# databendlabs/databend

Measured on AMD Instinct MI355X. Metric: rows/s TPC-H Q1 hash-agg, higher is better.
Workload: dtype i64/i128 decimal

## Files before the change

### databend_amd/csrc/gbk_merge_lds.h

```cpp

namespace {

int32_t ensure(void** p, size_t* cap, size_t bytes) {
  if (*cap >= bytes) return DBHIP_OK;
  if (*p) {
    int32_t rc = dbhip_free(*p);
    if (rc) return rc;
    *p = nullptr; *cap = 0;
  }
  size_t want = bytes + (bytes >> 3) + 256;
  int32_t rc = dbhip_alloc(want, p);
  if (rc) { *p = nullptr; return rc; }
  *cap = want;
  return DBHIP_OK;
}

int32_t alloc_table(dbhip_groupby* g, int64_t cap, hipStream_t s) {
  uint64_t* nh = nullptr;
  uint64_t* nr = nullptr;
  int32_t rc = dbhip_alloc((size_t)cap * 8, (void**)&nh);
  if (rc == DBHIP_OK) rc = dbhip_alloc((size_t)cap * g->L.W * 8, (void**)&nr);
  hipError_t e = rc == DBHIP_OK ? hipMemsetAsync(nh, 0, (size_t)cap * 8, s) : hipSuccess;
  if (rc != DBHIP_OK || e != hipSuccess) {
    if (nh) (void)dbhip_free(nh);
// ... 79 lines not shown
  const size_t need = (size_t)(used + extra);
  if (need <= g->arena_cap) return DBHIP_OK;
  size_t want = g->arena_cap ? g->arena_cap * 2 : ((size_t)1 << 20);
  while (want < need) want *= 2;
  uint8_t* na = nullptr;
  int32_t rc = dbhip_alloc(want, (void**)&na);
  if (rc) return rc;
  if (used) DBHIP_CHECK(hipMemcpyAsync(na, g->arena, (size_t)used, hipMemcpyDeviceToDevice, s));
  if (g->arena && layout_has_str_minmax(g->L))
    hipLaunchKernelGGL(gb_pin_strings_kernel, dim3(grid_for(g->cap, 256)), dim3(256), 0, s, g->L, g->slot_hash, g->rows, g->cap,
                       (uint64_t)g->arena, (uint64_t)g->arena + g->arena_cap, 2, na, (int64_t)((intptr_t)na - (intptr_t)g->arena), g->ctrl,
                       (unsigned long long*)nullptr);
  DBHIP_CHECK(hipStreamSynchronize(s));
  if (g->arena) (void)dbhip_free(g->arena);
  g->arena = na;
  g->arena_cap = want;
  return DBHIP_OK;
}
int32_t pin_string_states(dbhip_groupby* g, hipStream_t s) {
  if (!layout_has_str_minmax(g->L)) return DBHIP_OK;
  unsigned long long* acc = (unsigned long long*)&g->ctrl[10];
  DBHIP_CHECK(hipMemsetAsync(acc, 0, 8, s));
  const int grid = grid_for(g->cap, 256);
  hipLaunchKernelGGL(gb_pin_strings_kernel, dim3(grid), dim3(256), 0, s, g->L, g->slot_hash, g->rows, g->cap, (uint64_t)g->arena,
                     (uint64_t)g->arena + g->arena_cap, 0, g->arena, (int64_t)0, g->ctrl, acc);
  DBHIP_LAUNCH_CHECK();
  uint64_t bytes = 0;
  DBHIP_CHECK(hipMemcpyAsync(&bytes, acc, 8, hipMemcpyDeviceToHost, s));
  DBHIP_CHECK(hipStreamSynchronize(s));
  if (bytes == 0) return DBHIP_OK;
  int32_t rc = reserve_arena(g, bytes, s);
  if (rc) return rc;
  hipLaunchKernelGGL(gb_pin_strings_kernel, dim3(grid), dim3(256), 0, s, g->L, g->slot_hash, g->rows, g->cap, (uint64_t)g->arena,
                     (uint64_t)g->arena + g->arena_cap, 1, g->arena, (int64_t)0, g->ctrl, acc);
  DBHIP_LAUNCH_CHECK();
  g->arena_pinned += bytes;
  if (g->arena_pinned < (g->arena_live > ((uint64_t)1 << 20) ? g->arena_live : ((uint64_t)1 << 20))) return DBHIP_OK;
  g->arena_pinned = 0;
  DBHIP_CHECK(hipMemsetAsync(acc, 0, 8, s));
  hipLaunchKernelGGL(gb_pin_strings_kernel, dim3(grid), dim3(256), 0, s, g->L, g->slot_hash, g->rows, g->cap, (uint64_t)g->arena,
                     (uint64_t)g->arena + g->arena_cap, 3, g->arena, (int64_t)0, g->ctrl, acc);
  DBHIP_LAUNCH_CHECK();
  uint64_t two[2] = {0, 0};
  DBHIP_CHECK(hipMemcpyAsync(&two[0], acc, 8, hipMemcpyDeviceToHost, s));
  DBHIP_CHECK(hipMemcpyAsync(&two[1], &g->ctrl[8], 8, hipMemcpyDeviceToHost, s));
  DBHIP_CHECK(hipStreamSynchronize(s));
  g->arena_live = two[0];
  if (two[1] <= 2 * two[0] + ((uint64_t)1 << 20)) return DBHIP_OK;
  size_t want = (size_t)1 << 20;
  while (want < 2 * two[0]) want *= 2;
  uint8_t* na = nullptr;
  if ((rc = dbhip_alloc(want, (void**)&na))) return rc;
  DBHIP_CHECK(hipMemsetAsync(&g->ctrl[8], 0, 8, s));
  hipLaunchKernelGGL(gb_pin_strings_kernel, dim3(grid), dim3(256), 0, s, g->L, g->slot_hash, g->rows, g->cap, (uint64_t)g->arena,
                     (uint64_t)g->arena + g->arena_cap, 4, na, (int64_t)0, g->ctrl, acc);
  DBHIP_LAUNCH_CHECK();
  DBHIP_CHECK(hipStreamSynchronize(s));
  trace("groupby: string arena compacted, %llu bytes in use -> %llu live (capacity %zu -> %zu)",
        (unsigned long long)two[1], (unsigned long long)two[0], g->arena_cap, want);
  (void)dbhip_free(g->arena);
  g->arena = na;
  g->arena_cap = want;
  return DBHIP_OK;
}
int32_t reserve_arena_for_chunk(dbhip_groupby* g, hipStream_t s) {
  uint64_t lb = 0;
  DBHIP_CHECK(hipMemcpyAsync(&lb, &g->ctrl[9], 8, hipMemcpyDeviceToHost, s));
  DBHIP_CHECK(hipStreamSynchronize(s));
  if (lb == 0) return DBHIP_OK;
  g->has_long = 1;
  return reserve_arena(g, lb, s);
}
bool layout_has_strings(const GbLayout& L) { return L.str_w1_mask != 0; }
bool layout_has_wide_minmax(const GbLayout& L);

int32_t merge_rows_unpinned(dbhip_groupby* g, const uint64_t* rows_in, int64_t n, hipStream_t s, const uint64_t* n_dev, const uint64_t* abort_dev,
                            int deferred = 0);
int32_t merge_rows(dbhip_groupby* g, const uint64_t* rows_in, int64_t n, hipStream_t s,
                   const uint64_t* n_dev = nullptr, const uint64_t* abort_dev = nullptr) {
  int32_t rc = merge_rows_unpinned(g, rows_in, n, s, n_dev, abort_dev);
  if (rc == DBHIP_OK && n > 0) rc = pin_string_states(g, s);
  return rc;
}
int32_t merge_rows_unpinned(dbhip_groupby* g, const uint64_t* rows_in, int64_t n, hipStream_t s,
                            const uint64_t* n_dev, const uint64_t* abort_dev, int deferred) {
  if (n == 0) return DBHIP_OK;
  if (n > 0xFFFFFFF0LL) {
    set_error("groupby: more than 2^32 rows in one call");
    return DBHIP_ERR_INVALID;
  }
  int32_t rc;
  if ((rc = ensure((void**)&g->gid, &g->gid_cap, (size_t)n * 4))) return rc;
  if ((rc = ensure((void**)&g->retry, &g->retry_cap, (size_t)n * 4))) return rc;
  const int grid = grid_for(n, 256);
  uint64_t* host_ctrl = pinned_words(0);
  if (!host_ctrl) return DBHIP_ERR_HIP;
  const uint64_t* cur_rows = rows_in;
  int64_t cur_n = n;
  const DevCount dc{n_dev, abort_dev};
  if ((deferred || (g->count_host + n) * 135 <= g->cap * 100) && n <= 256) {
    hipLaunchKernelGGL(gb_merge_small_kernel, dim3(1), dim3(256), 0, s, g->L, cur_rows, cur_n, g->slot_hash, g->rows, g->cap, g->hash_mask, g->gid,
                       g->retry, g->ctrl, dc, g->arena);
    DBHIP_LAUNCH_CHECK();
    if (deferred) return DBHIP_OK;
    DBHIP_CHECK(hipMemcpyAsync(host_ctrl, g->ctrl, 5 * sizeof(uint64_t), hipMemcpyDeviceToHost, s));
    DBHIP_CHECK(hipStreamSynchronize(s));
    g->count_host = (int64_t)host_ctrl[0];
    if (host_ctrl[3] & 2) {
      set_error("groupby: a string key longer than 12 bytes was met; keep the CPU operator for this block");
      return DBHIP_ERR_UNSUPPORTED;
    }
    if (host_ctrl[1]) {
      set_error("groupby: collision chain filled the table during retry; create the table with a larger capacity");
      return DBHIP_ERR_CAPACITY;
    }
    return DBHIP_OK;
  }
  if (deferred || (g->count_host + n) * 135 <= g->cap * 100) {
    DBHIP_CHECK(hipMemsetAsync(&g->ctrl[1], 0, 16, s));
    hipLaunchKernelGGL(gb_probe_kernel, dim3(grid), dim3(256), 0, s, g->L, cur_rows, cur_n, g->slot_hash, g->rows, g->cap,
                       g->hash_mask, g->gid, g->ctrl, dc, g->arena);
    if (deferred == 1 || (!deferred && g->count_host > 0 && g->count_host <= 32 && n <= 65536) || n <= 2048 || layout_has_wide_minmax(g->L))
      hipLaunchKernelGGL(gb_accum_lowcard_kernel, dim3(deferred == 1 && grid > 16 ? 16 : grid), dim3(256), 0, s, g->L, cur_rows, cur_n, g->rows, g->gid, g->retry,
                         g->ctrl, dc, g->arena);
    else
      hipLaunchKernelGGL(gb_accum_kernel, dim3(grid), dim3(256), 0, s, g->L, cur_rows, cur_n, g->rows, g->gid, g->retry, g->ctrl, dc, g->arena);
    hipLaunchKernelGGL(gb_retry_kernel, dim3(1), dim3(64), 0, s, g->L, cur_rows, g->slot_hash, g->rows, g->cap, g->hash_mask,
                       g->gid, g->retry, g->ctrl, g->arena);
    DBHIP_LAUNCH_CHECK();
    if (deferred) return DBHIP_OK;
    DBHIP_CHECK(hipMemcpyAsync(host_ctrl, g->ctrl, 5 * sizeof(uint64_t), hipMemcpyDeviceToHost, s));
    DBHIP_CHECK(hipStreamSynchronize(s));
    g->count_host = (int64_t)host_ctrl[0];
    if (host_ctrl[3] & 2) {
      set_error("groupby: a string key longer than 12 bytes was met; keep the CPU operator for this block");
      return DBHIP_ERR_UNSUPPORTED;
    }
    if (host_ctrl[1]) {
      set_error("groupby: collision chain filled the table during retry; create the table with a larger capacity");
      return DBHIP_ERR_CAPACITY;
    }
    return DBHIP_OK;
  }
  if (n_dev || abort_dev) {
    set_error("groupby: device-side row count needs a table that cannot grow during the merge");
    return DBHIP_ERR_INVALID;
  }
  for (int attempt = 0; attempt < 40; ++attempt) {
    DBHIP_CHECK(hipMemsetAsync(&g->ctrl[1], 0, 16, s));
    hipLaunchKernelGGL(gb_probe_kernel, dim3(grid), dim3(256), 0, s, g->L, cur_rows, cur_n, g->slot_hash,
                       g->rows, g->cap, g->hash_mask, g->gid, g->ctrl, dc, g->arena);
    DBHIP_LAUNCH_CHECK();
    DBHIP_CHECK(hipMemcpyAsync(host_ctrl, g->ctrl, 5 * sizeof(uint64_t), hipMemcpyDeviceToHost, s));
    DBHIP_CHECK(hipStreamSynchronize(s));
    bool too_full = host_ctrl[1] != 0 || (int64_t)host_ctrl[0] * 135 > g->cap * 100;
    if (too_full) {
      if ((rc = grow(g, s))) return rc;
      continue;
    }
    g->count_host = (int64_t)host_ctrl[0];
    if (g->count_host <= 32 || layout_has_wide_minmax(g->L)) {
      hipLaunchKernelGGL(gb_accum_lowcard_kernel, dim3(grid), dim3(256), 0, s, g->L, cur_rows, cur_n,
                         g->rows, g->gid, g->retry, g->ctrl, dc, g->arena);
    } else {
      hipLaunchKernelGGL(gb_accum_kernel, dim3(grid), dim3(256), 0, s, g->L, cur_rows, cur_n, g->rows,
                         g->gid, g->retry, g->ctrl, dc, g->arena);
    }
    hipLaunchKernelGGL(gb_retry_kernel, dim3(1), dim3(64), 0, s, g->L, cur_rows, g->slot_hash, g->rows,
                       g->cap, g->hash_mask, g->gid, g->retry, g->ctrl, g->arena);
    DBHIP_LAUNCH_CHECK();
    DBHIP_CHECK(hipMemcpyAsync(host_ctrl, g->ctrl, 5 * sizeof(uint64_t), hipMemcpyDeviceToHost, s));
    DBHIP_CHECK(hipStreamSynchronize(s));
    g->count_host = (int64_t)host_ctrl[0];
    if (host_ctrl[3] & 2) {
      set_error("groupby: a string key longer than 12 bytes was met; keep the CPU operator for this block");
      return DBHIP_ERR_UNSUPPORTED;
    }
    if (host_ctrl[1] & 2) {
      set_error("groupby: collision chain filled the table during retry; create the table with a larger capacity");
      return DBHIP_ERR_CAPACITY;
    }
    return DBHIP_OK;
// ... 264 lines not shown
```

### databend_amd/csrc/gbk_rows.h

```cpp

namespace {

struct HashCols {
  GbCol c[GB_MAX_KEYS];
  int n;
};

__global__ __launch_bounds__(256) void group_hash_kernel(HashCols hc, int64_t n, uint64_t* out,
                                                         unsigned long long* bad) {
  constexpr int U = 4;
  const int64_t T = (int64_t)gridDim.x * blockDim.x;
  const int64_t t = (int64_t)blockIdx.x * blockDim.x + threadIdx.x;
  for (int64_t base = 0; base < n; base += U * T) {
    int64_t row[U];
    bool in[U];
    uint64_t h[U];
#pragma unroll
    for (int u = 0; u < U; ++u) {
      row[u] = base + u * T + t;
      in[u] = row[u] < n;
      if (!in[u]) row[u] = n - 1;
      h[u] = 0;
    }
    for (int k = 0; k < hc.n; ++k) {
// ... 163 lines not shown
      if (C.arg[a].data != nullptr && C.arg[a].type == DBHIP_T_STRING) {
        const GbCol& ac = C.arg[a];
#pragma unroll
        for (int u = 0; u < U; ++u) {
          const int64_t j = ac.is_scalar ? 0 : row[u];
          valid[u] = !ac.validity || bit_get(ac.validity, ac.voff + j);
          const uint32_t* v = (const uint32_t*)ac.data + 4 * j;
          const uint32_t len = v[0];
          uint64_t ww[2] = {0, 0};
          if (sv_is_inline(len) || !valid[u]) {
            bool vv;
            gb_load_words(ac, row[u], ww, &vv);
          } else if (ac.buffers) {
            ww[0] = ((uint64_t)v[1] << 32) | len;
            ww[1] = (uint64_t)sv_bytes(v, ac.buffers);
          } else {
            atomicOr((unsigned long long*)&ctrl[3], 2ULL);
          }
          w0[u] = ww[0]; w1[u] = ww[1];
        }
      } else if (C.arg[a].data != nullptr) gb_load_words_n<U>(C.arg[a], row, w0, w1, valid);
#pragma unroll
      for (int u = 0; u < U; ++u) {
        if (!in[u]) continue;
        uint64_t* s = rows_in + li[u] * L.W + L.agg_off[a];
        uint64_t v[GB_MAX_STATE_WORDS];
        gb_row_contrib(L, a, w0[u], w1[u], valid[u], v);
        for (int k = 0; k < L.agg_words[a]; ++k) s[k] = v[k];
      }
    }
  }
}

__device__ __forceinline__ uint64_t probe_word(uint64_t h, uint64_t mask) {
  uint64_t hw = h & mask;
  return hw == 0 ? 1 : hw;
}
__device__ __forceinline__ uint64_t home_slot(uint64_t hw, int64_t cap) {
  return hw >> (__builtin_clzll((unsigned long long)cap) + 1);
}

struct DevCount {
  const uint64_t* n_dev;
  const uint64_t* abort_dev;
};
__device__ __forceinline__ int64_t dev_rows(const DevCount& dc, int64_t n) {
  if (dc.abort_dev && (*dc.abort_dev & 7)) return 0;
  if (dc.n_dev) { const int64_t m = (int64_t)*dc.n_dev; return m < n ? m : n; }
  return n;
}

__device__ __forceinline__ bool bytes_equal(const uint8_t* x, const uint8_t* y, uint32_t len) {
  for (uint32_t i = 0; i < len; ++i)
    if (x[i] != y[i]) return false;
  return true;
}
__device__ __forceinline__ bool keys_equal(const GbLayout& L, const uint64_t* a, const uint64_t* b, const uint8_t* arena) {
  bool eq = true;
  for (int k = 0; k < L.nkey_words; ++k) {
    if (((L.str_w1_mask >> k) & 1) && (uint32_t)a[k - 1] > SV_INLINE_MAX) {
      eq = eq && a[k - 1] == b[k - 1] && bytes_equal((const uint8_t*)a[k], arena + b[k], (uint32_t)a[k - 1]);
      continue;
    }
    eq &= (a[k] == b[k]);
  }
  return eq;
}
__device__ __forceinline__ void write_group_keys(const GbLayout& L, const uint64_t* r, uint64_t* d, uint8_t* arena, uint64_t* ctrl) {
  for (int k = 0; k < L.nkey_words; ++k) {
    if (((L.str_w1_mask >> k) & 1) && (uint32_t)r[k - 1] > SV_INLINE_MAX) {
      const uint32_t len = (uint32_t)r[k - 1];
      const unsigned long long off = atomicAdd((unsigned long long*)&ctrl[8], (unsigned long long)((len + 7) & ~7u));
      const uint8_t* src = (const uint8_t*)r[k];
      for (uint32_t i = 0; i < len; ++i) arena[off + i] = src[i];
      d[k] = off;
      continue;
    }
    d[k] = r[k];
  }
}

__device__ __forceinline__ void gb_probe_body(const GbLayout& L, const uint64_t* rows_in, int64_t n,
                                              uint64_t* slot_hash, uint64_t* rows, int64_t cap,
                                              uint64_t hash_mask, uint32_t* gid, uint64_t* ctrl, uint8_t* arena) {
  const uint64_t cmask = (uint64_t)cap - 1;
  __shared__ uint32_t wg_new;
  if (threadIdx.x == 0) wg_new = 0;
  __syncthreads();
  uint32_t my_new = 0;
  for (int64_t i = (int64_t)blockIdx.x * blockDim.x + threadIdx.x; i < n;
       i += (int64_t)gridDim.x * blockDim.x) {
    bool claimed = false;
    {
      const uint64_t* r = rows_in + i * L.W;
      const uint64_t hw = probe_word(r[L.hash_word], hash_mask);
      uint64_t pos = home_slot(hw, cap);
      uint32_t found = GB_INVALID_SLOT;
      for (int64_t step = 0; step < cap; ++step) {
        unsigned long long cur = __hip_atomic_load((unsigned long long*)&slot_hash[pos], __ATOMIC_RELAXED,
                                                   __HIP_MEMORY_SCOPE_AGENT);
        if (cur == 0) {
          unsigned long long old = atomicCAS((unsigned long long*)&slot_hash[pos], 0ULL, (unsigned long long)hw);
          if (old == 0) {
            uint64_t* d = rows + pos * L.W;
            write_group_keys(L, r, d, arena, ctrl);
            d[L.hash_word] = r[L.hash_word];
            for (int a = 0; a < L.naggs; ++a) gb_state_identity(L, a, d + L.agg_off[a]);
            claimed = true;
            found = (uint32_t)pos;
            break;
          }
          cur = old;
        }
        if (cur == hw) {
          found = (uint32_t)pos;
          break;
        }
        pos = (pos + 1) & cmask;
      }
      if (found == GB_INVALID_SLOT) atomicOr((unsigned long long*)&ctrl[1], 1ULL);
      gid[i] = found;
    }
    my_new += claimed;
  }
  my_new = (uint32_t)wave_sum_u64(my_new);
  if (lane_id() == 0 && my_new) atomicAdd(&wg_new, my_new);
  __syncthreads();
  if (threadIdx.x == 0 && wg_new) atomicAdd((unsigned long long*)&ctrl[0], (unsigned long long)wg_new);
}
__global__ __launch_bounds__(256) void gb_probe_kernel(GbLayout L, const uint64_t* rows_in, int64_t n,
                                                       uint64_t* slot_hash, uint64_t* rows, int64_t cap,
                                                       uint64_t hash_mask, uint32_t* gid, uint64_t* ctrl, DevCount dc, uint8_t* arena) {
  gb_probe_body(L, rows_in, dev_rows(dc, n), slot_hash, rows, cap, hash_mask, gid, ctrl, arena);
}

__global__ __launch_bounds__(256) void gb_accum_kernel(GbLayout L, const uint64_t* rows_in, int64_t n,
                                                       uint64_t* rows, const uint32_t* gid,
                                                       uint32_t* retry, uint64_t* ctrl, DevCount dc, const uint8_t* arena) {
  n = dev_rows(dc, n);
  for (int64_t i = (int64_t)blockIdx.x * blockDim.x + threadIdx.x; i < n;
       i += (int64_t)gridDim.x * blockDim.x) {
    const uint64_t* r = rows_in + i * L.W;
    uint32_t pos = gid[i];
    uint64_t* d = rows + (uint64_t)pos * L.W;
    if (!keys_equal(L, r, d, arena)) {
      unsigned long long k = atomicAdd((unsigned long long*)&ctrl[2], 1ULL);
      retry[k] = (uint32_t)i;
      continue;
    }
    for (int a = 0; a < L.naggs; ++a) gb_atomic_merge(L, a, d + L.agg_off[a], r + L.agg_off[a]);
  }
}

__device__ __forceinline__ uint64_t wave_min_u64(uint64_t v) {
#pragma unroll
  for (int off = 32; off >= 1; off >>= 1) {
    uint64_t o = __shfl_xor(v, off, 64);
    v = o < v ? o : v;
  }
  return v;
}
__device__ __forceinline__ uint64_t wave_max_u64(uint64_t v) {
#pragma unroll
  for (int off = 32; off >= 1; off >>= 1) {
    uint64_t o = __shfl_xor(v, off, 64);
    v = o > v ? o : v;
  }
  return v;
}
__device__ __forceinline__ double wave_sum_f64(double v) {
#pragma unroll
  for (int off = 32; off >= 1; off >>= 1) v += __shfl_xor(v, off, 64);
  return v;
}

__device__ __forceinline__ void gb_accum_lowcard_body(const GbLayout& L, const uint64_t* rows_in,
                                                      int64_t n, uint64_t* rows,
                                                      const uint32_t* gid, uint32_t* retry,
                                                      uint64_t* ctrl, const uint8_t* arena) {
  const int64_t n_pad = (n + 63) & ~63LL;
  for (int64_t i = (int64_t)blockIdx.x * blockDim.x + threadIdx.x; i < n_pad;
       i += (int64_t)gridDim.x * blockDim.x) {
    bool active = i < n;
    const uint64_t* r = rows_in + (active ? i : 0) * L.W;
    uint32_t pos = active ? gid[i] : GB_INVALID_SLOT;
    if (active) {
      const uint64_t* d = rows + (uint64_t)pos * L.W;
      if (!keys_equal(L, r, d, arena)) {
        unsigned long long k = atomicAdd((unsigned long long*)&ctrl[2], 1ULL);
        retry[k] = (uint32_t)i;
        active = false;
      }
    }
    uint64_t todo = __ballot(active);
    while (todo) {
      int leader = __ffsll((long long)todo) - 1;
      uint32_t lpos = __shfl(pos, leader, 64);
      bool mine = active && pos == lpos;
      uint64_t m = __ballot(mine);
      uint64_t* d = rows + (uint64_t)lpos * L.W;
      for (int a = 0; a < L.naggs; ++a) {
        const uint64_t* v = r + L.agg_off[a];
        uint64_t out[GB_MAX_STATE_WORDS] = {0, 0, 0, 0};
        if (gb_minmax_str(L, a)) {
          if (mine) gb_minmax_str_locked(L.agg_kind[a] == DBHIP_AGG_MIN, d + L.agg_off[a], v);
          continue;
        }
        if (gb_sum256(L, a) || gb_minmax256(L, a)) {
          if (mine) gb_atomic_merge(L, a, d + L.agg_off[a], v);
          continue;
        }
        switch (L.agg_kind[a]) {
          case DBHIP_AGG_COUNT:
            out[0] = wave_sum_u64(mine ? v[0] : 0);
            break;
          case DBHIP_AGG_SUM:
            if (L.agg_flag[a]) out[L.agg_flag[a]] = wave_max_u64(mine ? v[L.agg_flag[a]] : 0);
            if (L.agg_words[a] - (L.agg_flag[a] ? 1 : 0) == 3) {
              u128 t = mine ? (((u128)v[1] << 64) | v[0]) : (u128)0;
              uint64_t e = mine ? v[2] : 0;
#pragma unroll
              for (int off = 32; off >= 1; off >>= 1) {
                uint64_t olo = __shfl_xor((uint64_t)t, off, 64), ohi = __shfl_xor((uint64_t)(t >> 64), off, 64);
                uint64_t oe = __shfl_xor(e, off, 64);
                u128 o = ((u128)ohi << 64) | olo;
                u128 r = t + o;
                e += oe + (r < t ? 1 : 0);
                t = r;
              }
              out[0] = (uint64_t)t;
              out[1] = (uint64_t)(t >> 64);
              out[2] = e;
            } else if (L.agg_type[a] == DBHIP_T_F32 || L.agg_type[a] == DBHIP_T_F64) {
              out[0] = (uint64_t)__double_as_longlong(
                  wave_sum_f64(mine ? __longlong_as_double((long long)v[0]) : 0.0));
            } else {
              out[0] = wave_sum_u64(mine ? v[0] : 0);
            }
            break;
          case DBHIP_AGG_MIN:
            out[0] = wave_min_u64((mine && v[1]) ? v[0] : ~0ULL);
            out[1] = wave_max_u64(mine ? v[1] : 0);
            if (L.agg_words[a] == 3) out[2] = wave_min_u64((mine && v[1] && v[0] == out[0]) ? v[2] : ~0ULL);
            break;
          default:
            out[0] = wave_max_u64((mine && v[1]) ? v[0] : 0ULL);
            out[1] = wave_max_u64(mine ? v[1] : 0);
            if (L.agg_words[a] == 3) out[2] = wave_max_u64((mine && v[1] && v[0] == out[0]) ? v[2] : 0ULL);
            break;
        }
        if (lane_id() == leader) gb_atomic_merge(L, a, d + L.agg_off[a], out);
      }
      todo &= ~m;
    }
  }
}
__global__ __launch_bounds__(256) void gb_accum_lowcard_kernel(GbLayout L, const uint64_t* rows_in,
                                                               int64_t n, uint64_t* rows,
                                                               const uint32_t* gid, uint32_t* retry,
                                                               uint64_t* ctrl, DevCount dc, const uint8_t* arena) {
  gb_accum_lowcard_body(L, rows_in, dev_rows(dc, n), rows, gid, retry, ctrl, arena);
}

__device__ __forceinline__ void gb_retry_body(const GbLayout& L, const uint64_t* rows_in, uint64_t* slot_hash, uint64_t* rows,
                                              int64_t cap, uint64_t hash_mask, const uint32_t* gid,
                                              const uint32_t* retry, uint64_t* ctrl, uint8_t* arena) {
  const uint64_t cmask = (uint64_t)cap - 1;
  const uint64_t nretry = ctrl[2];
  for (uint64_t t = 0; t < nretry; ++t) {
    const uint32_t i = retry[t];
    const uint64_t* r = rows_in + (uint64_t)i * L.W;
    const uint64_t hw = probe_word(r[L.hash_word], hash_mask);
    uint64_t pos = ((uint64_t)gid[i] + 1) & cmask;
    bool done = false;
    for (int64_t step = 0; step < cap && !done; ++step) {
      uint64_t cur = slot_hash[pos];
      uint64_t* d = rows + pos * L.W;
      if (cur == 0) {
        if ((int64_t)(ctrl[0] + 1) * 135 > cap * 100) break;
        slot_hash[pos] = hw;
        write_group_keys(L, r, d, arena, ctrl);
        d[L.hash_word] = r[L.hash_word];
        for (int a = 0; a < L.naggs; ++a) gb_state_identity(L, a, d + L.agg_off[a]);
        ctrl[0] += 1;
        cur = hw;
      }
      if (cur == hw && keys_equal(L, r, d, arena)) {
        for (int a = 0; a < L.naggs; ++a) gb_atomic_merge(L, a, d + L.agg_off[a], r + L.agg_off[a]);
        done = true;
      }
      pos = (pos + 1) & cmask;
    }
    if (!done) ctrl[1] |= 2;
  }
}
__global__ void gb_retry_kernel(GbLayout L, const uint64_t* rows_in, uint64_t* slot_hash, uint64_t* rows,
                                int64_t cap, uint64_t hash_mask, const uint32_t* gid,
                                const uint32_t* retry, uint64_t* ctrl, uint8_t* arena) {
  if (threadIdx.x != 0 || blockIdx.x != 0) return;
  gb_retry_body(L, rows_in, slot_hash, rows, cap, hash_mask, gid, retry, ctrl, arena);
}

__global__ __launch_bounds__(256) void gb_merge_small_kernel(GbLayout L, const uint64_t* rows_in, int64_t n, uint64_t* slot_hash, uint64_t* rows,
                                                             int64_t cap, uint64_t hash_mask, uint32_t* gid, uint32_t* retry, uint64_t* ctrl,
                                                             DevCount dc, uint8_t* arena) {
  n = dev_rows(dc, n);
  if (threadIdx.x < 2) ctrl[1 + threadIdx.x] = 0;
  __threadfence();
  __syncthreads();
  gb_probe_body(L, rows_in, n, slot_hash, rows, cap, hash_mask, gid, ctrl, arena);
  __threadfence();
  __syncthreads();
  gb_accum_lowcard_body(L, rows_in, n, rows, gid, retry, ctrl, arena);
  __threadfence();
  __syncthreads();
  if (threadIdx.x == 0) gb_retry_body(L, rows_in, slot_hash, rows, cap, hash_mask, gid, retry, ctrl, arena);
}

__global__ __launch_bounds__(256) void gb_rehash_kernel(GbLayout L, const uint64_t* old_hash,
                                                        const uint64_t* old_rows, int64_t old_cap,
                                                        uint64_t* new_hash, uint64_t* new_rows,
                                                        int64_t new_cap, uint64_t hash_mask) {
  const uint64_t cmask = (uint64_t)new_cap - 1;
  for (int64_t s = (int64_t)blockIdx.x * blockDim.x + threadIdx.x; s < old_cap;
       s += (int64_t)gridDim.x * blockDim.x) {
    uint64_t hw = old_hash[s];
    if (hw == 0) continue;
    const uint64_t* r = old_rows + s * L.W;
    uint64_t pos = home_slot(probe_word(r[L.hash_word], hash_mask), new_cap);
    while (true) {
      unsigned long long old = atomicCAS((unsigned long long*)&new_hash[pos], 0ULL, (unsigned long long)hw);
      if (old == 0) break;
      pos = (pos + 1) & cmask;
    }
    uint64_t* d = new_rows + pos * L.W;
    for (int k = 0; k < L.W; ++k) d[k] = r[k];
  }
}

__global__ __launch_bounds__(256) void gb_flush_kernel(GbLayout L, const uint64_t* slot_hash,
                                                       const uint64_t* rows, int64_t cap,
                                                       uint64_t* out_rows, int64_t max_rows, uint64_t* ctrl) {
  __shared__ uint32_t wtot[4];
  __shared__ unsigned long long base_s;
  const int tid = threadIdx.x, lane = tid & 63, wave = tid >> 6;
  const int64_t nchunks = (cap + 2047) / 2048;
  for (int64_t c = blockIdx.x; c < nchunks; c += gridDim.x) {
    const int64_t s0 = c * 2048 + (int64_t)tid * 8;
    uint32_t occ = 0;
#pragma unroll
    for (int k = 0; k < 8; ++k)
      if (s0 + k < cap && slot_hash[s0 + k] != 0) occ |= 1u << k;
    const uint32_t mine = (uint32_t)__popc(occ);
    uint32_t incl = mine;
#pragma unroll
    for (int d = 1; d < 64; d <<= 1) { const uint32_t o = __shfl_up(incl, d, 64); if (lane >= d) incl += o; }
    if (lane == 63) wtot[wave] = incl;
    __syncthreads();
    uint32_t wbase = 0, all = 0;
#pragma unroll
    for (int w = 0; w < 4; ++w) { if (w < wave) wbase += wtot[w]; all += wtot[w]; }
    if (tid == 0 && all) base_s = atomicAdd((unsigned long long*)&ctrl[4], (unsigned long long)all);
    __syncthreads();
    if (all) {
      uint64_t idx = base_s + wbase + incl - mine;
#pragma unroll
      for (int k = 0; k < 8; ++k) {
        if (!((occ >> k) & 1)) continue;
        if ((int64_t)idx < max_rows) {
          const uint64_t* r = rows + (s0 + k) * L.W;
          uint64_t* d = out_rows + idx * L.W;
          for (int q = 0; q < L.W; ++q) d[q] = r[q];
        }
        ++idx;
      }
    }
    __syncthreads();
  }
}

__global__ __launch_bounds__(64) void gb_block_header_kernel(uint64_t* block, int W, int64_t max_rows, const uint64_t* ctrl) {
  const int t = threadIdx.x;
  if (t < W) block[t] = t == 0 ? ((int64_t)ctrl[4] > max_rows ? ~0ULL : ctrl[4]) : 0;
}

__global__ __launch_bounds__(256) void gb_compact_blocks_kernel(const uint64_t* __restrict__ blocks, int64_t stride_words, int W,
                                                                int skip, uint64_t* __restrict__ out, uint64_t* __restrict__ xst = nullptr,
                                                                int n_blocks = 0, int64_t max_rows = 0, int check_w1 = 0) {
  const int b = blockIdx.x;
  if (xst) {
    uint64_t total = 0;
    int bad = 0;
    for (int p = 0; p < n_blocks; ++p) {
      const uint64_t c = blocks[(int64_t)p * stride_words];
      if (c == ~0ULL || (int64_t)c > max_rows || (check_w1 && blocks[(int64_t)p * stride_words + 1] != 0)) { if (!bad) bad = p + 1; }
      else if (p != skip) total += c;
    }
    if (b == 0 && threadIdx.x == 0) { xst[0] = bad ? 0 : total; xst[1] = bad ? 1 : 0; xst[2] = (uint64_t)bad; }
    if (bad) return;
// ... 433 lines not shown
```

### databend_amd/csrc/k_fagg.hip

```cpp
#include "fagg_device.h"
#include "runtime.h"

#include <dirent.h>
#include <dlfcn.h>
#include <errno.h>
#include <sys/stat.h>
#include <fcntl.h>
#include <signal.h>
#include <spawn.h>
#include <sys/wait.h>
#include <unistd.h>

#include <atomic>
#include <chrono>
#include <deque>
#include <map>
#include <mutex>
#include <string>

#include <stdlib.h>
#include <string.h>
#include <time.h>

using namespace dbhip;
// ... 875 lines not shown
    }
    put(prog->arg_regs, (size_t)L.naggs * 4);
    const char hf = filter_bitmap != nullptr;
    put(&hf, 1);
    int sh = -1;
    for (int i = (int)pp->shapes.size() - 1; i >= 0 && sh < 0; --i)
      if (pp->shapes[(size_t)i].sig == sig) sh = i;
    if (sh < 0) {
      FaShape S;
      FaArgs A;
      memset(&A, 0, sizeof(A));
      bool may_raise = false;
      const int32_t rc = fa_build_args(L, keys, prog, A, &S.general, &S.nwords, &may_raise);
      if (rc) return rc;
      A.has_filter = filter_bitmap != nullptr;
      S.lds = (size_t)(A.P.n_slots > 6 ? A.P.n_slots : 6) * FA_ROWS * 256 * 8;
      if (S.lds > 60 * 1024) {
        set_error("dbhip_groupby_add_block_program: %d live LDS slots exceed the register file; split the expression", A.P.n_slots);
        return DBHIP_ERR_UNSUPPORTED;
      }
      fa_shape(A, S.A);
      S.sig = sig;
      pp->shapes.push_back(std::move(S));
      sh = (int)pp->shapes.size() - 1;
    }
    FaPending P;
    memset(&P.b, 0, sizeof(P.b));
    P.shape = sh;
    for (int c = 0; c < prog->n_inputs; ++c) {
      P.b.in_data[c] = prog->inputs[c].data; P.b.in_valid[c] = prog->inputs[c].validity; P.b.in_voff[c] = prog->inputs[c].validity_offset;
    }
    for (int k = 0; k < L.nkeys; ++k) { P.b.key_data[k] = keys[k].data; P.b.key_valid[k] = keys[k].validity; P.b.key_voff[k] = keys[k].validity_offset; }
    P.b.filter_bits = filter_bitmap; P.b.filter_off = filter_bit_offset; P.b.n = n;
    pp->bound = true; pp->stream = s;
    return fa_pipe_enqueue(g, pp, P, s);
  }
  FaArgs A;
  memset(&A, 0, sizeof(A));
  bool general = false, may_raise = false;
  int nwords = 0;
  int32_t rc = fa_build_args(L, keys, prog, A, &general, &nwords, &may_raise);
  if (rc) return rc;
  A.filter_bits = filter_bitmap; A.filter_off = filter_bit_offset; A.n = n;
  A.has_filter = filter_bitmap != nullptr;
  const size_t lds = (size_t)(A.P.n_slots > 6 ? A.P.n_slots : 6) * FA_ROWS * 256 * 8;
  if (lds > 60 * 1024) {
    set_error("dbhip_groupby_add_block_program: %d live LDS slots exceed the register file; split the expression", A.P.n_slots);
    return DBHIP_ERR_UNSUPPORTED;
  }
  const int64_t nchunks = ceil_div(n, 64 * FA_ROWS);
  const int grid = (int)(ceil_div(nchunks, 4) < 512 ? ceil_div(nchunks, 4) : 512);
  if (FaPipe* pp = (FaPipe*)*dbhip_groupby_pipe_slot_internal(g); pp && !t_prepare_only) {
    int64_t committed = 0;
    if ((rc = fa_pipe_checkpoint(g, pp, &committed, true))) return rc;
  }
  const size_t rows_bytes = (size_t)grid * FA_MAX_SLOTS * L.W * 8;
  uint8_t* ws = (uint8_t*)scratch(rows_bytes + 64, 6, s);
  if (!ws) return DBHIP_ERR_HIP;
  uint64_t* ctrl = (uint64_t*)ws;
  A.ctrl = ctrl;
  A.partial_rows = (uint64_t*)(ws + 64);
  A.P.err_words = nullptr;
  A.P.err_count = (unsigned long long*)&ctrl[2];
  uint64_t* host_ctrl = pinned_words(1);
  if (!host_ctrl) return DBHIP_ERR_HIP;
  host_ctrl[0] = host_ctrl[1] = host_ctrl[2] = 0;
  const int64_t n_max = (int64_t)grid * FA_MAX_SLOTS;
  const bool chained = (dbhip_groupby_count_internal(g) + n_max) * 135 <= dbhip_groupby_capacity_internal(g) * 100;
  if ((rc = dbhip_groupby_reserve_merge_internal(g, n_max))) return rc;
  if (t_prepare_only) {
    (void)jit_kernel(A, dbhip_groupby_count_internal(g) > 4 ? 8 : 4, general, nwords, JIT_COMPILE);
    if (FaPipe* pq = (FaPipe*)*dbhip_groupby_pipe_slot_internal(g); pq && pq->on)
      (void)jit_kernel(A, dbhip_groupby_count_internal(g) > 4 ? 8 : 4, general, nwords, JIT_COMPILE, nullptr, true);
    return DBHIP_OK;
  }
  for (int variant = dbhip_groupby_count_internal(g) > 4 ? 1 : 0; variant < 2; ++variant) {
    DBHIP_CHECK(hipMemsetAsync(ctrl, 0, 64, s));
    kernel_timer_start(s);
    if ((rc = fa_launch(A, variant == 0 ? 4 : 8, general, nwords, grid, lds, s))) return rc;
    kernel_timer_stop(s);
    DBHIP_LAUNCH_CHECK();
    DBHIP_CHECK(hipMemcpyAsync(host_ctrl, ctrl, 24, hipMemcpyDeviceToHost, s));
    if (chained && !may_raise) {
      rc = dbhip_groupby_merge_rows_dev_internal(g, A.partial_rows, n_max, &ctrl[0], &ctrl[1], s);
      if (rc) return rc;
      if (!(host_ctrl[1] & 3)) return DBHIP_OK;
    } else {
      DBHIP_CHECK(hipStreamSynchronize(s));
    }
    if (!(host_ctrl[1] & 1)) break;
  }
  if (host_ctrl[1] & 2) {
    set_error("dbhip_groupby_add_block_program: a group key string is longer than 12 bytes");
    return DBHIP_ERR_UNSUPPORTED;
  }
  if (host_ctrl[1] & 1) {
    set_error("dbhip_groupby_add_block_program: more than %d distinct groups inside one workgroup; use the operator-at-a-time path", FA_MAX_SLOTS);
    return DBHIP_ERR_CAPACITY;
  }
  if (host_ctrl[2]) {
    set_error("dbhip_groupby_add_block_program: %llu row error(s) in the fused maps (Decimal overflow / divided by zero); "
              "evaluate the maps with dbhip_expr_eval to get the rows", (unsigned long long)host_ctrl[2]);
    return DBHIP_ERR_ROW_ERRORS;
  }
  return dbhip_groupby_merge_rows_internal(g, A.partial_rows, (int64_t)host_ctrl[0], s);
}

int32_t dbhip_groupby_set_pipelined(dbhip_groupby* g, int32_t on, void* stream) {
  DBHIP_REQUIRE(g, "dbhip_groupby_set_pipelined: NULL argument");
  void** slot = dbhip_groupby_pipe_slot_internal(g);
  FaPipe* pp = (FaPipe*)*slot;
  if (!on) {
    if (!pp) return DBHIP_OK;
    int64_t committed = 0;
    const int32_t rc = fa_pipe_checkpoint(g, pp, &committed, true);
    pp->on = false; pp->bound = false;
    return rc;
  }
  const GbLayout& L = *dbhip_groupby_layout_internal(g);
  if (!dbhip_fagg_layout_ok_internal(L)) {
    set_error("dbhip_groupby_set_pipelined: layout outside the fused kernel (<= %d key words, <= %d aggregates, <= %d state words)", FA_KW, FA_MAXA, FA_MAXW);
    return DBHIP_ERR_UNSUPPORTED;
  }
  if (pp) { pp->on = true; return DBHIP_OK; }
  pp = new (std::nothrow) FaPipe();
  DBHIP_REQUIRE(pp, "dbhip_groupby_set_pipelined: out of host memory");
  hipStream_t s = resolve_stream(stream);
  pp->cap_rows = 65536;
  int32_t rc = dbhip_alloc((size_t)pp->cap_rows * L.W * 8, (void**)&pp->rows);
  hipError_t e = rc == DBHIP_OK ? hipMalloc((void**)&pp->ctrl, 64) : hipSuccess;
  if (rc == DBHIP_OK && e == hipSuccess) e = hipHostMalloc((void**)&pp->status_host, 64, hipHostMallocMapped);
  if (rc == DBHIP_OK && e == hipSuccess) e = hipHostGetDevicePointer((void**)&pp->status_dev, pp->status_host, 0);
  if (rc == DBHIP_OK && e == hipSuccess) { memset(pp->status_host, 0, 64); e = hipMemsetAsync(pp->ctrl, 0, 64, s); }
  if (rc == DBHIP_OK && e == hipSuccess) e = hipStreamSynchronize(s);
  for (int i = 0; i < FA_PIPE_RING && rc == DBHIP_OK && e == hipSuccess; ++i) {
    e = hipHostMalloc((void**)&pp->tab_host[i], FA_PIPE_TABLE_BYTES, hipHostMallocDefault);
    if (e == hipSuccess) e = hipMalloc((void**)&pp->tab_dev[i], FA_PIPE_TABLE_BYTES);
    if (e == hipSuccess) e = hipEventCreateWithFlags(&pp->tab_ev[i], hipEventDisableTiming);
  }
  if (rc == DBHIP_OK && e == hipSuccess) rc = dbhip_groupby_reserve_merge_internal(g, pp->cap_rows);
  if (rc != DBHIP_OK || e != hipSuccess) {
    dbhip_fagg_pipe_destroy_internal(pp);
    return rc != DBHIP_OK ? rc : hip_fail(e, "dbhip_groupby_set_pipelined");
  }
  pp->count_seen = dbhip_groupby_count_internal(g);
  pp->on = true;
  *slot = pp;
  return DBHIP_OK;
}

int32_t dbhip_groupby_checkpoint(dbhip_groupby* g, int64_t* out_blocks_committed_host, void* stream) {
  DBHIP_REQUIRE(g, "dbhip_groupby_checkpoint: NULL argument");
  if (out_blocks_committed_host) *out_blocks_committed_host = 0;
  FaPipe* pp = (FaPipe*)*dbhip_groupby_pipe_slot_internal(g);
  if (!pp) return DBHIP_OK;
  if (pp->bound && stream && pp->stream != resolve_stream(stream)) {
    set_error("dbhip_groupby_checkpoint: the table's blocks were queued on another stream");
    return DBHIP_ERR_INVALID;
  }
  const int32_t rc = fa_pipe_checkpoint(g, pp, out_blocks_committed_host, true);
  pp->bound = false;
  return rc;
}

int32_t dbhip_groupby_prepare_program(dbhip_groupby* g, const dbhip_col* keys, const dbhip_agg_program* prog) {
  t_prepare_only = true;
  const int32_t rc = dbhip_groupby_add_block_program(g, keys, prog, 1, nullptr, 0, nullptr);
// ... 146 lines not shown
```

Measured before the change: 89.07 billion.

## Add LDS fold-merge kernel that pre-aggregates partial rows before global hash merge

Adds a single-workgroup merge kernel with 1024 threads. It first folds the incoming partial rows into a small LDS hash table, word by word with LDS atomics, then probes and accumulates only the distinct folded groups (plus any unfolded overflow rows) into the global hash table. This is meant to replace many global atomic merges on few groups with cheap LDS atomics, and it prefetches input words into registers. The chained fused-agg path also passes a tighter row bound for the 4-slot variant. The cost is more kernel complexity, a large LDS footprint, and carry-propagation logic for multiword sums.

New measurement: 89.31 billion (median of 6 runs). No clear change (+0.3%).

```diff
diff --git a/databend_amd/csrc/gbk_merge_lds.h b/databend_amd/csrc/gbk_merge_lds.h
--- a/databend_amd/csrc/gbk_merge_lds.h
+++ b/databend_amd/csrc/gbk_merge_lds.h
@@ -185,6 +185,31 @@
   if (rc == DBHIP_OK && n > 0) rc = pin_string_states(g, s);
   return rc;
 }
+struct FmShape { int lcap, n_cap; size_t lds; };
+bool fold_merge_shape(const GbLayout& L, int64_t n, FmShape* out) {
+  if (n > FM_MAX_ROWS || layout_has_wide_minmax(L)) return false;
+  int lcap = 256;
+  while (lcap >= 8 && (size_t)lcap * L.W * 8 > 40 * 1024) lcap >>= 1;
+  if (lcap < 8) return false;
+  out->lcap = lcap;
+  out->n_cap = (int)n;
+  out->lds = 8 * ((size_t)lcap * L.W + 2 * (size_t)lcap) + 4 * ((size_t)((L.W + 1) & ~1) + (size_t)lcap) + 2 * (2 * (size_t)lcap + 2 * (size_t)((n + 3) & ~3LL));
+  return out->lds <= 60 * 1024;
+}
+int32_t merge_read_back(dbhip_groupby* g, uint64_t* host_ctrl, hipStream_t s) {
+  DBHIP_CHECK(hipMemcpyAsync(host_ctrl, g->ctrl, 5 * sizeof(uint64_t), hipMemcpyDeviceToHost, s));
+  DBHIP_CHECK(hipStreamSynchronize(s));
+  g->count_host = (int64_t)host_ctrl[0];
+  if (host_ctrl[3] & 2) {
+    set_error("groupby: a string key longer than 12 bytes was met; keep the CPU operator for this block");
+    return DBHIP_ERR_UNSUPPORTED;
+  }
+  if (host_ctrl[1]) {
+    set_error("groupby: collision chain filled the table during retry; create the table with a larger capacity");
+    return DBHIP_ERR_CAPACITY;
+  }
+  return DBHIP_OK;
+}
 int32_t merge_rows_unpinned(dbhip_groupby* g, const uint64_t* rows_in, int64_t n, hipStream_t s,
                             const uint64_t* n_dev, const uint64_t* abort_dev, int deferred) {
   if (n == 0) return DBHIP_OK;
@@ -201,6 +226,14 @@
   const uint64_t* cur_rows = rows_in;
   int64_t cur_n = n;
   const DevCount dc{n_dev, abort_dev};
+  FmShape fm;
+  if ((deferred || (g->count_host + n) * 135 <= g->cap * 100) && fold_merge_shape(g->L, n, &fm)) {
+    hipLaunchKernelGGL(gb_fold_merge_kernel, dim3(1), dim3(FM_THREADS), fm.lds, s, g->L, cur_rows, cur_n, g->slot_hash, g->rows, g->cap, g->hash_mask,
+                       g->gid, g->retry, g->ctrl, dc, g->arena, fm.lcap, fm.n_cap);
+    DBHIP_LAUNCH_CHECK();
+    if (deferred) return DBHIP_OK;
+    return merge_read_back(g, host_ctrl, s);
+  }
   if ((deferred || (g->count_host + n) * 135 <= g->cap * 100) && n <= 256) {
     hipLaunchKernelGGL(gb_merge_small_kernel, dim3(1), dim3(256), 0, s, g->L, cur_rows, cur_n, g->slot_hash, g->rows, g->cap, g->hash_mask, g->gid,
                        g->retry, g->ctrl, dc, g->arena);
diff --git a/databend_amd/csrc/gbk_rows.h b/databend_amd/csrc/gbk_rows.h
--- a/databend_amd/csrc/gbk_rows.h
+++ b/databend_amd/csrc/gbk_rows.h
@@ -269,7 +269,8 @@
 
 __device__ __forceinline__ void gb_probe_body(const GbLayout& L, const uint64_t* rows_in, int64_t n,
                                               uint64_t* slot_hash, uint64_t* rows, int64_t cap,
-                                              uint64_t hash_mask, uint32_t* gid, uint64_t* ctrl, uint8_t* arena) {
+                                              uint64_t hash_mask, uint32_t* gid, uint64_t* ctrl, uint8_t* arena,
+                                              const uint16_t* idx = nullptr) {
   const uint64_t cmask = (uint64_t)cap - 1;
   __shared__ uint32_t wg_new;
   if (threadIdx.x == 0) wg_new = 0;
@@ -279,7 +280,7 @@
        i += (int64_t)gridDim.x * blockDim.x) {
     bool claimed = false;
     {
-      const uint64_t* r = rows_in + i * L.W;
+      const uint64_t* r = rows_in + (idx ? (int64_t)idx[i] : i) * L.W;
       const uint64_t hw = probe_word(r[L.hash_word], hash_mask);
       uint64_t pos = home_slot(hw, cap);
       uint32_t found = GB_INVALID_SLOT;
@@ -321,13 +322,11 @@
   gb_probe_body(L, rows_in, dev_rows(dc, n), slot_hash, rows, cap, hash_mask, gid, ctrl, arena);
 }
 
-__global__ __launch_bounds__(256) void gb_accum_kernel(GbLayout L, const uint64_t* rows_in, int64_t n,
-                                                       uint64_t* rows, const uint32_t* gid,
-                                                       uint32_t* retry, uint64_t* ctrl, DevCount dc, const uint8_t* arena) {
-  n = dev_rows(dc, n);
+__device__ __forceinline__ void gb_accum_body(const GbLayout& L, const uint64_t* rows_in, int64_t n, uint64_t* rows, const uint32_t* gid,
+                                              uint32_t* retry, uint64_t* ctrl, const uint8_t* arena, const uint16_t* idx = nullptr) {
   for (int64_t i = (int64_t)blockIdx.x * blockDim.x + threadIdx.x; i < n;
        i += (int64_t)gridDim.x * blockDim.x) {
-    const uint64_t* r = rows_in + i * L.W;
+    const uint64_t* r = rows_in + (idx ? (int64_t)idx[i] : i) * L.W;
     uint32_t pos = gid[i];
     uint64_t* d = rows + (uint64_t)pos * L.W;
     if (!keys_equal(L, r, d, arena)) {
@@ -337,6 +336,11 @@
     }
     for (int a = 0; a < L.naggs; ++a) gb_atomic_merge(L, a, d + L.agg_off[a], r + L.agg_off[a]);
   }
+}
+__global__ __launch_bounds__(256) void gb_accum_kernel(GbLayout L, const uint64_t* rows_in, int64_t n,
+                                                       uint64_t* rows, const uint32_t* gid,
+                                                       uint32_t* retry, uint64_t* ctrl, DevCount dc, const uint8_t* arena) {
+  gb_accum_body(L, rows_in, dev_rows(dc, n), rows, gid, retry, ctrl, arena);
 }
 
 __device__ __forceinline__ uint64_t wave_min_u64(uint64_t v) {
@@ -451,12 +455,12 @@
 
 __device__ __forceinline__ void gb_retry_body(const GbLayout& L, const uint64_t* rows_in, uint64_t* slot_hash, uint64_t* rows,
                                               int64_t cap, uint64_t hash_mask, const uint32_t* gid,
-                                              const uint32_t* retry, uint64_t* ctrl, uint8_t* arena) {
+                                              const uint32_t* retry, uint64_t* ctrl, uint8_t* arena, const uint16_t* idx = nullptr) {
   const uint64_t cmask = (uint64_t)cap - 1;
   const uint64_t nretry = ctrl[2];
   for (uint64_t t = 0; t < nretry; ++t) {
     const uint32_t i = retry[t];
-    const uint64_t* r = rows_in + (uint64_t)i * L.W;
+    const uint64_t* r = rows_in + (uint64_t)(idx ? (uint32_t)idx[i] : i) * L.W;
     const uint64_t hw = probe_word(r[L.hash_word], hash_mask);
     uint64_t pos = ((uint64_t)gid[i] + 1) & cmask;
     bool done = false;
@@ -502,6 +506,190 @@
   __threadfence();
   __syncthreads();
   if (threadIdx.x == 0) gb_retry_body(L, rows_in, slot_hash, rows, cap, hash_mask, gid, retry, ctrl, arena);
+}
+
+enum { FM_SKIP = 0, FM_ADD, FM_ADDC, FM_FADD, FM_MIN, FM_MAX, FM_OR };
+constexpr uint32_t FM_NONE = 0xFFFFu;
+constexpr int FM_THREADS = 1024;
+constexpr int64_t FM_MAX_ROWS = 4096;
+
+__device__ __forceinline__ void gb_accum_spread_body(const GbLayout& L, const uint64_t* rows_in, int64_t n, uint64_t* rows, const uint32_t* gid,
+                                                     uint32_t* retry, uint64_t* ctrl, const uint8_t* arena, const uint16_t* idx,
+                                                     uint32_t* any_retry) {
+  const int na = L.naggs > 0 ? L.naggs : 1;
+  const int64_t total = n * na;
+  for (int64_t x = threadIdx.x; x < total; x += blockDim.x) {
+    const int64_t i = x / na;
+    const int a = (int)(x - i * na);
+    const uint64_t* r = rows_in + (idx ? (int64_t)idx[i] : i) * L.W;
+    uint64_t* d = rows + (uint64_t)gid[i] * L.W;
+    if (!keys_equal(L, r, d, arena)) {
+      if (a == 0) {
+        unsigned long long k = atomicAdd((unsigned long long*)&ctrl[2], 1ULL);
+        retry[k] = (uint32_t)i;
+        *any_retry = 1;
+      }
+      continue;
+    }
+    if (a < L.naggs) gb_atomic_merge(L, a, d + L.agg_off[a], r + L.agg_off[a]);
+  }
+}
+
+__device__ __forceinline__ void gb_fold_merge_step(const GbLayout& L, const uint64_t* rows_in, int64_t n, const uint16_t* idx, uint64_t* slot_hash,
+                                                   uint64_t* rows, int64_t cap, uint64_t hash_mask, uint32_t* gid, uint32_t* retry,
+                                                   uint64_t* ctrl, uint8_t* arena, uint32_t* any_retry) {
+  gb_probe_body(L, rows_in, n, slot_hash, rows, cap, hash_mask, gid, ctrl, arena, idx);
+  __syncthreads();
+  gb_accum_spread_body(L, rows_in, n, rows, gid, retry, ctrl, arena, idx, any_retry);
+  __syncthreads();
+  if (threadIdx.x == 0 && *any_retry) {
+    __threadfence();
+    gb_retry_body(L, rows_in, slot_hash, rows, cap, hash_mask, gid, retry, ctrl, arena, idx);
+    ctrl[2] = 0;
+    *any_retry = 0;
+    __threadfence();
+  }
+  __syncthreads();
+}
+
+__device__ __forceinline__ uint64_t gb_fold_word(uint32_t op, uint64_t v, uint64_t* d, const uint64_t* seen) {
+  switch (op) {
+    case FM_ADD:
+      if (v) atomicAdd((unsigned long long*)d, (unsigned long long)v);
+      break;
+    case FM_ADDC:
+      if (v) return atomicAdd((unsigned long long*)d, (unsigned long long)v);
+      break;
+    case FM_FADD:
+      atomicAdd((double*)d, __longlong_as_double((long long)v));
+      break;
+    case FM_MIN:
+      if (*seen) atomicMin((unsigned long long*)d, (unsigned long long)v);
+      break;
+    case FM_MAX:
+      if (*seen) atomicMax((unsigned long long*)d, (unsigned long long)v);
+      break;
+    default:
+      if (v) atomicOr((unsigned long long*)d, 1ULL);
+      break;
+  }
+  return 0;
+}
+__device__ __forceinline__ void gb_fold_carry(uint64_t* d, const uint32_t* lop_w) {
+  for (;;) {
+    ++d; ++lop_w;
+    const uint64_t old = atomicAdd((unsigned long long*)d, 1ULL);
+    if (*lop_w != FM_ADDC || old != ~0ULL) break;
+  }
+}
+
+__global__ __launch_bounds__(FM_THREADS) void gb_fold_merge_kernel(GbLayout L, const uint64_t* __restrict__ rows_in, int64_t n_bound,
+                                                                   uint64_t* slot_hash, uint64_t* rows, int64_t cap, uint64_t hash_mask,
+                                                                   uint32_t* gid, uint32_t* retry, uint64_t* ctrl, DevCount dc, uint8_t* arena,
+                                                                   int lcap, int n_cap) {
+  extern __shared__ uint64_t fm_lds[];
+  __shared__ uint32_t lcount, lnpass, lretry;
+  constexpr int T = FM_THREADS;
+  const int W = L.W, tid = threadIdx.x;
+  uint64_t* lrows = fm_lds;
+  uint64_t* lhash = lrows + (size_t)lcap * W;
+  uint32_t* lop = (uint32_t*)(lhash + 2 * lcap);
+  uint32_t* lgid = lop + ((W + 1) & ~1);
+  uint16_t* lidx = (uint16_t*)(lgid + lcap);
+  uint16_t* eid = lidx + 2 * lcap;
+  uint16_t* pass = eid + n_cap;
+  const uint32_t hmask = 2u * (uint32_t)lcap - 1;
+  const uint32_t cap_words = (uint32_t)n_cap * (uint32_t)W;
+  uint64_t q0 = rows_in[(uint32_t)tid < cap_words ? tid : 0], q1 = rows_in[(uint32_t)(tid + T) < cap_words ? tid + T : 0];
+  uint64_t q2 = rows_in[(uint32_t)(tid + 2 * T) < cap_words ? tid + 2 * T : 0], q3 = rows_in[(uint32_t)(tid + 3 * T) < cap_words ? tid + 3 * T : 0];
+  int64_t n64 = dev_rows(dc, n_bound);
+  const int n = (int)(n64 < (int64_t)n_cap ? n64 : (int64_t)n_cap);
+  if (tid < 2) ctrl[1 + tid] = 0;
+  if (tid == 0) { lcount = 0; lnpass = 0; lretry = 0; }
+  for (int s = tid; s <= (int)hmask; s += T) lhash[s] = 0;
+  for (int w = tid; w < W; w += T) lop[w] = FM_SKIP;
+  __syncthreads();
+  for (int a = tid; a < L.naggs; a += T) {
+    const int off = L.agg_off[a], fw = L.agg_flag[a];
+    switch (L.agg_kind[a]) {
+      case DBHIP_AGG_COUNT:
+        lop[off] = FM_ADD;
+        break;
+      case DBHIP_AGG_SUM: {
+        const int ns = L.agg_words[a] - (fw ? 1 : 0);
+        if (L.agg_type[a] == DBHIP_T_F32 || L.agg_type[a] == DBHIP_T_F64) lop[off] = FM_FADD;
+        else for (int k = 0; k < ns; ++k) lop[off + k] = k + 1 < ns ? FM_ADDC : FM_ADD;
+        if (fw) lop[off + fw] = FM_OR;
+      } break;
+      case DBHIP_AGG_MIN:
+        lop[off] = FM_MIN; lop[off + 1] = FM_OR;
+        break;
+      default:
+        lop[off] = FM_MAX; lop[off + 1] = FM_OR;
+        break;
+    }
+  }
+  __syncthreads();
+
+#pragma nounroll
+  for (int base = 0; base < n; base += T) {
+    const int i = base + tid;
+    const uint64_t* r = rows_in + (size_t)(i < n ? i : 0) * W;
+    uint32_t slot = FM_NONE;
+    if (i < n) {
+      const uint64_t hw = probe_word(r[L.hash_word], hash_mask);
+      uint32_t pos = (uint32_t)(hw ^ (hw >> 29)) & hmask;
+      for (uint32_t step = 0; step <= hmask; ++step) {
+        uint64_t cur = ((volatile uint64_t*)lhash)[pos];
+        if (cur == 0) {
+          const unsigned long long old = atomicCAS((unsigned long long*)&lhash[pos], 0ULL, (unsigned long long)hw);
+          if (old == 0) {
+            const uint32_t e = atomicAdd(&lcount, 1u);
+            if (e < (uint32_t)lcap) {
+              uint64_t* d = lrows + (size_t)e * W;
+              for (int k = 0; k < L.nkey_words; ++k) d[k] = r[k];
+              d[L.hash_word] = r[L.hash_word];
+              for (int a = 0; a < L.naggs; ++a) gb_state_identity(L, a, d + L.agg_off[a]);
+            }
+            lidx[pos] = (uint16_t)(e < (uint32_t)lcap ? e : FM_NONE);
+            slot = pos;
+            break;
+          }
+          cur = old;
+        }
+        if (cur == hw) { slot = pos; break; }
+        pos = (pos + 1) & hmask;
+      }
+    }
+    __syncthreads();
+    if (i < n) {
+      uint32_t e = slot == FM_NONE ? FM_NONE : (uint32_t)lidx[slot];
+      if (e != FM_NONE && !keys_equal(L, r, lrows + (size_t)e * W, (const uint8_t*)0)) e = FM_NONE;
+      eid[i] = (uint16_t)e;
+      if (e == FM_NONE) pass[atomicAdd(&lnpass, 1u)] = (uint16_t)i;
+    }
+  }
+  __syncthreads();
+
+  const uint32_t total = (uint32_t)n * (uint32_t)W;
+#pragma nounroll
+  for (uint32_t f = tid; f < total; f += T) {
+    const uint64_t v = q0;
+    q0 = q1; q1 = q2; q2 = q3;
+    q3 = rows_in[f + 4 * T < cap_words ? f + 4 * T : 0];
+    const uint32_t row = f / (uint32_t)W, w = f - row * (uint32_t)W;
+    const uint32_t op = lop[w], e = eid[row];
+    if (op == FM_SKIP || e == FM_NONE) continue;
+    uint64_t* d = lrows + (size_t)e * W + w;
+    const uint64_t old = gb_fold_word(op, v, d, rows_in + f + 1);
+    if (op == FM_ADDC && old + v < v) gb_fold_carry(d, lop + w);
+  }
+  __syncthreads();
+
+  const int ne = (int)(lcount < (uint32_t)lcap ? lcount : (uint32_t)lcap);
+  const int np = (int)lnpass;
+  if (ne) gb_fold_merge_step(L, lrows, ne, nullptr, slot_hash, rows, cap, hash_mask, lgid, retry, ctrl, arena, &lretry);
+  if (np) gb_fold_merge_step(L, rows_in, np, pass, slot_hash, rows, cap, hash_mask, gid, retry, ctrl, arena, &lretry);
 }
 
 __global__ __launch_bounds__(256) void gb_rehash_kernel(GbLayout L, const uint64_t* old_hash,
diff --git a/databend_amd/csrc/k_fagg.hip b/databend_amd/csrc/k_fagg.hip
--- a/databend_amd/csrc/k_fagg.hip
+++ b/databend_amd/csrc/k_fagg.hip
@@ -981,7 +981,7 @@
     DBHIP_LAUNCH_CHECK();
     DBHIP_CHECK(hipMemcpyAsync(host_ctrl, ctrl, 24, hipMemcpyDeviceToHost, s));
     if (chained && !may_raise) {
-      rc = dbhip_groupby_merge_rows_dev_internal(g, A.partial_rows, n_max, &ctrl[0], &ctrl[1], s);
+      rc = dbhip_groupby_merge_rows_dev_internal(g, A.partial_rows, (int64_t)grid * (variant == 0 ? 4 : FA_MAX_SLOTS), &ctrl[0], &ctrl[1], s);
       if (rc) return rc;
       if (!(host_ctrl[1] & 3)) return DBHIP_OK;
     } else {
```
